# cboin1996/avddpg

Hardware: AMD Instinct MI355X
Metric: env-steps/sec + DDPG updates/sec, 4096x5-vehicle platoons (higher is better)
Workload: dtype f32-class (fp16 hi+lo operand pairs on the 16-bit matrix cores, f32 accumulate)

## Files before the change

### avddpg_amd/csrc/fsplit.hip

```cpp
#include <type_traits>

#include "fset_common.h"

namespace avd {
namespace fsplit {
using namespace fset;

struct ActorS {
    static constexpr int K = 256, KP = 256, NFT = 8, NKS = 16, LD = 264, NGT = 9, KG = 288;
    static constexpr bool critic = false;
};
struct CriticS {
    static constexpr int K = 304, KP = 320, NFT = 10, NKS = 19, LD = 312, NGT = 10, KG = 320;
    static constexpr bool critic = true;
};
constexpr int NGT_MAX = 10;

template <int I, int N, class F>
__device__ __forceinline__ void static_for(F&& f) {
    if constexpr (I < N) {
        f(std::integral_constant<int, I>{});
        static_for<I + 1, N>(f);
    }
}
// ... 17 lines not shown
    f32x2 l;
#ifdef __HIP_DEVICE_COMPILE__
    asm("v_fma_mix_f32 %0, -%1, 1.0, %2 op_sel:[0,0,0] op_sel_hi:[1,0,0]" : "=v"(l[0]) : "v"(hi), "v"(a));
    asm("v_fma_mix_f32 %0, -%1, 1.0, %2 op_sel:[1,0,0] op_sel_hi:[1,0,0]" : "=v"(l[1]) : "v"(hi), "v"(b));
#else
    l[0] = a - (float)h[0], l[1] = b - (float)h[1];
#endif
    lo = __builtin_bit_cast(unsigned, __builtin_convertvector(l, f16x2));
}
__device__ __forceinline__ void split1h(float x, f16& hi, f16& lo) {
    hi = (f16)x;
    lo = (f16)(x - (float)hi);
}
template <class V>
__device__ __forceinline__ void pin16(V& x) {
#pragma unroll
    for (int q = 0; q < 2; ++q) {
        float a = x[8 * q], b = x[8 * q + 1], c = x[8 * q + 2], d = x[8 * q + 3], e = x[8 * q + 4], f = x[8 * q + 5], g = x[8 * q + 6], h = x[8 * q + 7];
        asm volatile("" : "+v"(a), "+v"(b), "+v"(c), "+v"(d), "+v"(e), "+v"(f), "+v"(g), "+v"(h));
        x[8 * q] = a, x[8 * q + 1] = b, x[8 * q + 2] = c, x[8 * q + 3] = d, x[8 * q + 4] = e, x[8 * q + 5] = f, x[8 * q + 6] = g, x[8 * q + 7] = h;
    }
}
__device__ __forceinline__ f16x8 fragh(unsigned a, unsigned b, unsigned c, unsigned d) {
    uint4 o;
    o.x = a, o.y = b, o.z = c, o.w = d;
    return __builtin_bit_cast(f16x8, o);
}
__device__ __forceinline__ f32x16 mfmah(f16x8 a, f16x8 b, f32x16 c) {
    return __builtin_amdgcn_mfma_f32_32x32x16_f16(a, b, c, 0, 0, 0);
}
__device__ __forceinline__ f16x8 make_xh(float x0, float x1, float x2, float x3, int h) {
    f16 a0, a1, a2, a3, l0, l1, l2, l3;
    split1h(x0, a0, l0), split1h(x1, a1, l1), split1h(x2, a2, l2), split1h(x3, a3, l3);
    const f16 one = (f16)1.f, zero = (f16)0.f;
    f16x8 v;
    v[0] = a0, v[1] = a1, v[2] = a2, v[3] = a3;
    v[4] = h ? one : l0, v[5] = h ? one : l1, v[6] = h ? zero : l2, v[7] = h ? zero : l3;
    return v;
}
__device__ __forceinline__ f16x8 make_wh(float w0, float w1, float w2, float w3, float b, float sc, int h) {
    f16 a0, a1, a2, a3, l0, l1, l2, l3, bh, bl;
    split1h(sc * w0, a0, l0), split1h(sc * w1, a1, l1), split1h(sc * w2, a2, l2), split1h(sc * w3, a3, l3), split1h(sc * b, bh, bl);
    const f16 zero = (f16)0.f;
    f16x8 v;
    v[0] = h ? l0 : a0, v[1] = h ? l1 : a1, v[2] = h ? l2 : a2, v[3] = h ? l3 : a3;
    v[4] = h ? bh : a0, v[5] = h ? bl : a1, v[6] = h ? bh : a2, v[7] = h ? zero : a3;
    return v;
}
__device__ __forceinline__ f16x8 make_xg(float x0, float x1, float x2, float x3, float g, int h) {
    f16 a0, a1, a2, a3, l0, l1, l2, l3, gh, gl;
    split1h(x0, a0, l0), split1h(x1, a1, l1), split1h(x2, a2, l2), split1h(x3, a3, l3), split1h(g, gh, gl);
    const f16 zero = (f16)0.f;
    f16x8 v;
    v[0] = a0, v[1] = a1, v[2] = a2, v[3] = a3;
    v[4] = h ? gh : l0, v[5] = h ? gh : l1, v[6] = h ? gl : l2, v[7] = h ? zero : l3;
    return v;
}

template <int S>
__device__ __forceinline__ void load_x(const float* xa, long row, float (&x)[4]) {
    if (S == 4) {
        const float4 v = *(const float4*)(xa + 4 * row);
        x[0] = v.x, x[1] = v.y, x[2] = v.z, x[3] = v.w;
    } else {
#pragma unroll
        for (int k = 0; k < 4; ++k) x[k] = k < S ? xa[S * row + k] : 0.f;
    }
}

__host__ __device__ constexpr int wpos(int f) { return (f & ~12) | ((f & 4) << 1) | ((f & 8) >> 1); }

struct NetP {
    const float* th;
    long th_stride;
    const f16* Whi;
    const f16* Wlo;
    const f16* Wchi;
    const f16* Wclo;
    const f16x8* wf1h;
    const float* vec;
    const unsigned* wap;
};

struct PackArgs {
    const float* x[2];
    const float* extra[2];
    f16x8* outh[2];
    long rows;
};
__device__ __forceinline__ void front_flag(unsigned* wave_flags, bool hit) {
    const bool any = __ballot(hit) != 0;
    if ((threadIdx.x & 63) == 0) wave_flags[threadIdx.x >> 6] = any;
}
template <int S>
__device__ __forceinline__ void pack_x_role(const PackArgs& a, int which, long bx, unsigned* wave_flags) {
    const float* x = a.x[which];
    const float* extra = a.extra[which];
    const bool extra_is_action = which == 0;
    const long i = bx * 256 + threadIdx.x;
    bool nf = false;
    if (i < 2 * a.rows) {
        float v[4];
        load_x<S>(x, i >> 1, v);
        nf = not_finite(v[0]) || not_finite(v[1]) || not_finite(v[2]) || not_finite(v[3]);
        nf = nf || fmaxf(fmaxf(fabsf(v[0]), fabsf(v[1])), fmaxf(fabsf(v[2]), fabsf(v[3]))) >= F16_OVERFLOW;
        if (!(i & 1)) {
            const float e = extra[i >> 1];
            nf = nf || not_finite(e) || (extra_is_action && fabsf(e) >= F16_OVERFLOW);
        }
        a.outh[which][i] = make_xh(v[0], v[1], v[2], v[3], (int)(i & 1));
    }
    front_flag(wave_flags, nf);
}

struct PrepArgs {
    avd_mlp_layout L;
    int S;
    const float *theta, *stats, *theta_t, *stats_t;
    f16 *Whi[4], *Wlo[4];
    f16 *Wchi[4], *Wclo[4];
    f16x8* wf1h[4];
    float* vec[4];
    unsigned* wap;
    unsigned* smax;
    int* bad;
    unsigned* fflag;
    int n_fflag;
};
constexpr int SCALE_SLICES = 16;
__device__ __forceinline__ float pow2_for(float mx) {
    int e = 0;
    if (mx > 0.f && !not_finite(mx)) (void)frexpf(mx, &e);
    int k = 13 - e;
    k = k < -14 ? -14 : (k > 30 ? 30 : k);
    return ldexpf(1.f, k);
}
__device__ __forceinline__ void scale_role(const PrepArgs& a, int net, int set, int slice, int n_sets) {
    __shared__ float red[256], red2[256], c3a[H2], inva[CriticS::K];
    const int tid = threadIdx.x;
    const bool critic = net & 1, target = net >= 2;
    const avd_mlp_layout& L = a.L;
    const float* th = (target ? a.theta_t : a.theta) + (long)set * L.theta_size + (critic ? L.actor_size : 0);
    const float* st = (target ? a.stats_t : a.stats) + (long)set * L.stats_size;
    const int K = critic ? CriticS::K : ActorS::K, oW2 = critic ? L.cW2 : L.aW2;
    const int og2 = critic ? L.cg3 : L.ag2, omv2 = critic ? L.cmv3 : L.amv2, oW3 = critic ? L.cW3 : L.aW3;
    if (tid < H2) c3a[tid] = fabsf((1.0f / sqrtf(st[omv2 + tid] + BN_EPS)) * th[og2 + tid] * th[oW3 + tid]);
    for (int f = tid; f < K; f += 256) {
        int og, omv, ff = f;
        if (!critic) og = L.ag1, omv = L.amv1;
        else if (f < H1) og = L.cgs, omv = L.cmvs;
        else og = L.cga, omv = L.cmva, ff = f - H1;
        inva[f] = fabsf((1.0f / sqrtf(st[omv + ff] + BN_EPS)) * th[og + ff]);
    }
    __syncthreads();
    const int total = K * H2, per = (total + SCALE_SLICES - 1) / SCALE_SLICES, lo = slice * per, hi = min(total, lo + per);
    float m = 0.f, m2 = 0.f;
    for (int i = lo + tid; i < hi; i += 256) {
        const float w = fabsf(th[oW2 + i]);
        m = fmaxf(m, inva[i / H2] * w);
        m2 = fmaxf(m2, c3a[i % H2] * w);
    }
    red[tid] = m, red2[tid] = m2;
    __syncthreads();
    for (int o = 128; o > 0; o >>= 1) {
        if (tid < o) red[tid] = fmaxf(red[tid], red[tid + o]), red2[tid] = fmaxf(red2[tid], red2[tid + o]);
        __syncthreads();
    }
    if (tid == 0) {
        unsigned* dst = a.smax + (((long)net * n_sets + set) * SCALE_SLICES + slice) * 2;
        dst[0] = __float_as_uint(red[0]);
        dst[1] = __float_as_uint(red2[0]);
    }
}
__global__ __launch_bounds__(320) void prep_kernel(const PrepArgs a) {
    __shared__ float red[320];
    const int n = blockIdx.x, net = blockIdx.y, set = blockIdx.z, f = threadIdx.x;
    const bool critic = net & 1, target = net >= 2;
    const avd_mlp_layout& L = a.L;
    const float* th = (target ? a.theta_t : a.theta) + (long)set * L.theta_size + (critic ? L.actor_size : 0);
    const float* st = (target ? a.stats_t : a.stats) + (long)set * L.stats_size;
    const int K = critic ? CriticS::K : ActorS::K, KP = critic ? CriticS::KP : ActorS::KP;
    const int oW2 = critic ? L.cW2 : L.aW2, ob2 = critic ? L.cb2 : L.ab2, oW3 = critic ? L.cW3 : L.aW3, ob3 = critic ? L.cb3 : L.ab3;
    const int og2 = critic ? L.cg3 : L.ag2, obe2 = critic ? L.cbe3 : L.abe2, omm2 = critic ? L.cmm3 : L.amm2, omv2 = critic ? L.cmv3 : L.amv2;
    const float inv2n = (1.0f / sqrtf(st[omv2 + n] + BN_EPS)) * th[og2 + n], c3n = inv2n * th[oW3 + n];
    const unsigned* smax = a.smax + ((long)net * gridDim.z + set) * SCALE_SLICES * 2;
    unsigned mx = 0, mxc = 0;
#pragma unroll
    for (int sl = 0; sl < SCALE_SLICES; ++sl) mx = max(mx, smax[2 * sl]), mxc = max(mxc, smax[2 * sl + 1]);
    const float SW = pow2_for(__uint_as_float(mx)), SWC = pow2_for(__uint_as_float(mxc));
    if (net == 0 && set == 0)
        for (int w = n * 320 + f; w < a.n_fflag; w += H2 * 320)
            if (a.fflag[w]) atomicOr(a.bad, 1);
    float shw = 0.f;
    if (f < KP) {
        float w = 0.f, inv = 0.f;
// ... 15 lines not shown
            a.Whi[net][at] = hi, a.Wlo[net][at] = lo;
        }
        if (!target) {
            f16 hi, lo;
            const float wc = SWC * (c3n * w);
            if (fabsf(wc) >= F16_OVERFLOW) atomicOr(a.bad, 1);
            split1h(wc, hi, lo);
            const long at = ((long)set * KP + f) * H2 + n;
            a.Wchi[net][at] = hi, a.Wclo[net][at] = lo;
        }
    }
    red[f] = shw;
    __syncthreads();
    if (f < 64) red[f] += red[f + 256];
    __syncthreads();
    for (int o = 128; o > 0; o >>= 1) {
        if (f < o) red[f] += red[f + o];
        __syncthreads();
    }
    float* vec = a.vec[net] + (long)set * VEC;
    if (f == 0) {
        if (n == 0) vec[2 * H2 + 1] = SW, vec[2 * H2 + 2] = SWC;
        vec[n] = th[ob2 + n] + red[0];
        vec[H2 + n] = c3n;
        if (not_finite(vec[n]) || not_finite(c3n) || not_finite(th[ob3])) atomicOr(a.bad, 1);
    }
    if (n == 0) {
        __syncthreads();
        float v = 0.f;
        if (f < H2) {
            const float inv2 = (1.0f / sqrtf(st[omv2 + f] + BN_EPS)) * th[og2 + f];
            v = (th[obe2 + f] - st[omm2 + f] * inv2) * th[oW3 + f];
        }
        red[f] = v;
        __syncthreads();
        for (int o = 64; o > 0; o >>= 1) {
            if (f < o) red[f] += red[f + o];
            __syncthreads();
        }
        if (f == 0) vec[2 * H2] = th[ob3] + red[0];
    }
}
__device__ __forceinline__ bool prep1_role(const PrepArgs& a, int ft, int net, int set, int lane) {
    const int r = lane & 31, h = lane >> 5;
    bool hit = false;
    const bool critic = net & 1, target = net >= 2;
    const avd_mlp_layout& L = a.L;
    const float* th = (target ? a.theta_t : a.theta) + (long)set * L.theta_size + (critic ? L.actor_size : 0);
    const int K = critic ? CriticS::K : ActorS::K;
    const int f = 32 * ft + r;
    float w[4] = {0.f, 0.f, 0.f, 0.f}, b = 0.f;
    if (f == K) {
        b = 1.f;
    } else if (f < K) {
        if (critic && ft >= 8) {
            w[0] = th[L.cWa + (f - H1)], b = th[L.cba + (f - H1)];
        } else {
            const float* W = th + (critic ? L.cWs : L.aW1);
#pragma unroll
            for (int k = 0; k < 4; ++k) w[k] = k < a.S ? W[k * H1 + f] : 0.f;
            b = th[(critic ? L.cbs : L.ab1) + f];
        }
        if (not_finite(w[0]) || not_finite(w[1]) || not_finite(w[2]) || not_finite(w[3]) || not_finite(b)) hit = true;
        if (S1 * fmaxf(fmaxf(fabsf(w[0]), fabsf(w[1])), fmaxf(fmaxf(fabsf(w[2]), fabsf(w[3])), fabsf(b))) >= F16_OVERFLOW) hit = true;
    }
    a.wf1h[net][((long)set * NGT_MAX + ft) * 64 + lane] = make_wh(w[0], w[1], w[2], w[3], b, S1, h);
    if (net == 1 && ft == 0 && lane < 48) {
        const int hl = lane / 24, hh = (lane / 12) & 1, ks = (lane / 4) % 3, m = lane & 3;
        unsigned v = 0;
#pragma unroll
        for (int e = 0; e < 2; ++e) {
            const int jj = 2 * m + e, fa = 16 * ks + 8 * (jj >> 2) + 4 * hh + (jj & 3);
            f16 hi, lo;
            split1h(S1 * th[L.cWa + fa], hi, lo);
            v |= (unsigned)__builtin_bit_cast(unsigned short, hl ? lo : hi) << (16 * e);
        }
        a.wap[(long)set * 48 + lane] = v;
    }
    return hit;
}

struct FrontArgs {
    PrepArgs pa;
    PackArgs pk;
    float* grads;
    long n_grads;
    int n_sets, n_scale, n_prep1, n_zero, n_pack;
};
constexpr int ZERO_PER_BLOCK = 4096;
template <int S>
__global__ __launch_bounds__(256) void front_kernel(const FrontArgs a) {
    int b = blockIdx.x;
    if (b < a.n_scale) {
        scale_role(a.pa, b & 3, (b >> 2) % a.n_sets, (b >> 2) / a.n_sets, a.n_sets);
        return;
    }
    b -= a.n_scale;
    if (b < a.n_prep1) {
        const int q = 4 * b + (threadIdx.x >> 6);
        bool hit = false;
        if (q < NGT_MAX * 4 * a.n_sets) hit = prep1_role(a.pa, q % NGT_MAX, (q / NGT_MAX) & 3, q / (NGT_MAX * 4), threadIdx.x & 63);
        front_flag(a.pa.fflag + 4 * (long)b, hit);
        return;
    }
    b -= a.n_prep1;
    if (b < a.n_zero) {
        if (b == 0 && threadIdx.x == 0) *a.pa.bad = 0;
        const long base = (long)b * ZERO_PER_BLOCK + threadIdx.x;
#pragma unroll
        for (int k = 0; k < ZERO_PER_BLOCK / 256; ++k)
            if (base + 256 * k < a.n_grads) a.grads[base + 256 * k] = 0.f;
        return;
    }
    b -= a.n_zero;
    const int which = b >= a.n_pack;
    pack_x_role<S>(a.pk, which, b - which * a.n_pack, a.pa.fflag + 4 * ((long)a.n_prep1 + b));
}

enum HeadMode { OUT_TANH = 0, OUT_TD = 1, HEAD_BOTH = 5, OUT_TANH_SAVE = 6 };
struct HeadArgs {
    unsigned long long* stamp;
    NetP net;
    int n_agents, n_sets;
    const f16x8* xf;
    const float* act;
    const float* act2;
    const float* r;
    const float* yin;
    const float* aw;
    float* out;
    unsigned* sm;
    float* g3;
    float* dmu;
    float* part_s;
    float* part_s2;
    float* part_m;
    float* tz;
    float gamma, high, inv_n;
    int* bad;
    int abl;
};
#ifndef HEAD_FAST
#define HEAD_FAST 5
#define HEAD_SLOW 3
#endif

template <int S, class NET, int MODE, bool HP = false, class... H>
__global__ __launch_bounds__(NT) void head_kernel(const HeadArgs p, H... hp) {
    constexpr int K = NET::K, NKS = NET::NKS, NFT = NET::NFT, LD = NET::LD;
    constexpr int NTH = NT;
    constexpr bool BOTH = (MODE == HEAD_BOTH);
    static_assert(!BOTH || NET::critic, "HEAD_BOTH is a critic mode");
    __shared__ __attribute__((aligned(16))) f16 wimg[2][H2 * LD];
    __shared__ __attribute__((aligned(16))) float b2s[H2];
    __shared__ __attribute__((aligned(16))) float c3s[H2];
    __shared__ __attribute__((aligned(16))) unsigned waps[BOTH ? 48 : 4];
    const int tid = threadIdx.x, w = tid >> 6, lane = tid & 63, r = lane & 31, h = lane >> 5, q = w >> 1, rh = w & 1;
    const int set = blockIdx.x % p.n_sets, j0 = blockIdx.x / p.n_sets, J = gridDim.x / p.n_sets, P = p.n_agents / p.n_sets;
    for (int i = tid; i < 2 * H2 * (K / 8); i += NTH) {
        const int hl = i / (H2 * (K / 8)), rem = i - hl * (H2 * (K / 8)), n = rem / (K / 8), c = rem - n * (K / 8);
        const f16* src = (hl ? p.net.Wlo : p.net.Whi) + ((long)set * H2 + n) * K + 8 * c;
        *(uint4*)(&wimg[hl][n * LD + 8 * c]) = *(const uint4*)src;
    }
    const float* vec = p.net.vec + (long)set * VEC;
    const float SW = vec[2 * H2 + 1], sc = SW * S1, isc = 1.f / sc;
    if (tid < H2) b2s[tid] = vec[tid] * sc, c3s[tid] = vec[H2 + tid] * isc;
    if (BOTH && tid < 48) waps[tid] = p.net.wap[(long)set * 48 + tid];
    const float d3 = vec[2 * H2];
    const f16x8* wf1 = p.net.wf1h + (long)set * NGT_MAX * 64 + lane;
    const f32x16 zero16 = {};
#ifdef AVD_STAMP
    unsigned long long hacc[4] = {0, 0, 0, 0}, hlast = __builtin_amdgcn_s_memtime();
    const unsigned long long hstart = hlast;
#define HSTAMP(i) { const unsigned long long t_ = __builtin_amdgcn_s_memtime(); hacc[i] += t_ - hlast; hlast = t_; }
#else
#define HSTAMP(i)
#endif
    float Dacc = 0.f, Lacc = 0.f, Dacc2 = 0.f, Lacc2 = 0.f, gmax = 0.f;
    unsigned watch = 0;
    auto look = [&](float x) {
        unsigned u = __float_as_uint(x);
        asm volatile("" : "+v"(u));
        u &= 0x7fffffffu;
        watch = watch > u ? watch : u;
    };
    __syncthreads();

    const int ntile = j0 < P ? (P - j0 + J - 1) / J : 0;
    const int row = 32 * rh + r;
    f16x8 nx = {};
    float na = 0.f, nb = 0.f, ny = 0.f, nw = 1.f;
    auto fetch_in = [&](int k) {
        const int agent = (j0 + k * J) * p.n_sets + set;
        const long ri = (long)agent * TILE + row;
        nx = p.xf[2 * ri + h];
        if (NET::critic) na = p.act[ri];
        if (BOTH) nb = p.act2[ri];
        if (MODE == OUT_TD) ny = p.r[ri];
        if (BOTH) ny = p.yin[ri];
        if (BOTH && p.aw) nw = p.aw[agent];
    };
    const f16* whi0 = &wimg[0][r * LD + 8 * h];
    const f16* wlo0 = &wimg[1][r * LD + 8 * h];
    constexpr int NSEQ = BOTH ? 8 : NFT;
    HSTAMP(3);
    constexpr int FAST = HEAD_FAST, SLOW = HEAD_SLOW, PERIOD = 2 * (FAST + SLOW);
    const int qs = __builtin_amdgcn_readfirstlane(q);
    const int cnt = qs < 2 ? FAST : SLOW, start = qs < 2 ? qs * FAST : 2 * FAST + (qs - 2) * SLOW;
    int k = start, pos = 0;
    auto next_tile = [&](int kk, int pp) { return pp + 1 == cnt ? kk + PERIOD - cnt + 1 : kk + 1; };
    if (k < ntile) fetch_in(k);
    for (int ui = 0; k < ntile; ++ui, k = next_tile(k, pos), pos = pos + 1 == cnt ? 0 : pos + 1) {
        const int agent = (j0 + k * J) * p.n_sets + set;
        const long ri = (long)agent * TILE + row;
        const f16x8 xs = nx, xa = make_xh(na, 0.f, 0.f, 0.f, h), xb = BOTH ? make_xh(nb, 0.f, 0.f, 0.f, h) : xa;
        const float ty = ny, tw = nw;
        if (next_tile(k, pos) < ntile) fetch_in(next_tile(k, pos));
        f32x16 acc[4];
#pragma unroll
        for (int t = 0; t < 4; ++t)
#pragma unroll
            for (int g = 0; g < 4; ++g) {
                const float4 b = *(const float4*)(b2s + 32 * t + 8 * g + 4 * h);
                acc[t][4 * g] = b.x, acc[t][4 * g + 1] = b.y, acc[t][4 * g + 2] = b.z, acc[t][4 * g + 3] = b.w;
            }
        unsigned ph[8], pl[8];
        auto split16 = [&](const f32x16& p1) {
            if (FSPLIT_ABL(p.abl) & 4) {
#pragma unroll
                for (int m = 0; m < 8; ++m) ph[m] = __float_as_uint(p1[2 * m]), pl[m] = __float_as_uint(p1[2 * m + 1]);
                return;
            }
#pragma unroll
            for (int m = 0; m < 8; ++m) split2h(relu(p1[2 * m]), relu(p1[2 * m + 1]), ph[m], pl[m]);
        };
        auto zdot_t = [&](f32x16& a, int t) {
            float zp = 0.f;
#pragma unroll
            for (int g = 0; g < 4; ++g) {
                const float4 c = *(const float4*)(c3s + 32 * t + 8 * g + 4 * h);
                const float cc[4] = {c.x, c.y, c.z, c.w};
#pragma unroll
                for (int j = 0; j < 4; ++j) {
                    a[4 * g + j] = relu(a[4 * g + j]);
                    zp = fmaf(a[4 * g + j], cc[j], zp);
                }
            }
            return zp;
        };
        auto zdot_nd = [&](const f32x16& a, int t) {
            float zp = 0.f;
#pragma unroll
            for (int g = 0; g < 4; ++g) {
                const float4 c = *(const float4*)(c3s + 32 * t + 8 * g + 4 * h);
                const float cc[4] = {c.x, c.y, c.z, c.w};
#pragma unroll
                for (int j = 0; j < 4; ++j) zp = fmaf(relu(a[4 * g + j]), cc[j], zp);
            }
            return zp;
        };
        auto mask_t = [&](const f32x16& a) {
            unsigned b = 0;
#pragma unroll
            for (int g = 0; g < 4; ++g)
#pragma unroll
                for (int j = 0; j < 4; ++j) b |= a[4 * g + j] > 0.f ? 1u << (4 * g + (j >> 1) + 16 * (j & 1)) : 0u;
            return b;
        };
        auto mask_store = [&](const unsigned (&b)[4], unsigned* dst) {
            const auto s0 = __builtin_amdgcn_permlane32_swap(b[0], b[2], false, false);
            const auto s1 = __builtin_amdgcn_permlane32_swap(b[1], b[3], false, false);
            uint2 o;
            o.x = s0[0] | (s0[1] << 2), o.y = s1[0] | (s1[1] << 2);
            *(uint2*)(dst + 2 * h) = o;
        };
        auto out_z = [&](f32x16 (&ac)[4]) {
            float zp = 0.f;
#pragma unroll
            for (int t = 0; t < 4; ++t) zp += zdot_t(ac[t], t);
            zp += __shfl_xor(zp, 32);
            return d3 + zp;
        };
        split16(mfmah(wf1[0], xs, zero16));
        f16x8 wfn = wf1[64];
        f16x8 wg[2][2][2];
        auto read_group = [&](int g, f16x8 (&dst)[2][2]) {
            const int ks = g >> 1, th = g & 1;
#pragma unroll
            for (int tt = 0; tt < 2; ++tt) {
                dst[tt][0] = *(const f16x8*)(whi0 + 32 * (2 * th + tt) * LD + 16 * ks);
                dst[tt][1] = *(const f16x8*)(wlo0 + 32 * (2 * th + tt) * LD + 16 * ks);
            }
        };
        read_group(0, wg[0]);
        auto tile = [&](auto si_c, f32x16 (&ac)[4]) {
            constexpr int si = decltype(si_c)::value;
            constexpr int ft = si;
            f32x16 p1n = zero16;
// ... 82 lines not shown
            }
            __builtin_amdgcn_sched_barrier(0);
            f16x8 mh[3], ml[3];
#pragma unroll
            for (int tl = 0; tl < 2; ++tl) {
                const f32x16 pa = mfmah(wf1[64 * (8 + tl)], xa, zero16), pm = mfmah(wf1[64 * (8 + tl)], xb, zero16);
                unsigned dh[8], dl[8], mk[8];
#pragma unroll
                for (int m = 0; m < 4 * (2 - tl); ++m) {
                    split2h(relu(pm[2 * m]) - relu(pa[2 * m]), relu(pm[2 * m + 1]) - relu(pa[2 * m + 1]), dh[m], dl[m]);
                    mk[m] = (pm[2 * m] > 0.f ? 0xffffu : 0u) | (pm[2 * m + 1] > 0.f ? 0xffff0000u : 0u);
                }
#pragma unroll
                for (int ss = 0; ss < 2 - tl; ++ss) {
                    const int kk = 2 * tl + ss;
                    fh[kk] = fragh(dh[4 * ss], dh[4 * ss + 1], dh[4 * ss + 2], dh[4 * ss + 3]);
                    fl[kk] = fragh(dl[4 * ss], dl[4 * ss + 1], dl[4 * ss + 2], dl[4 * ss + 3]);
                    const uint4 ch = *(const uint4*)(waps + (0 * 2 + h) * 12 + 4 * kk), cl = *(const uint4*)(waps + (1 * 2 + h) * 12 + 4 * kk);
                    mh[kk] = fragh(ch.x & mk[4 * ss], ch.y & mk[4 * ss + 1], ch.z & mk[4 * ss + 2], ch.w & mk[4 * ss + 3]);
                    ml[kk] = fragh(cl.x & mk[4 * ss], cl.y & mk[4 * ss + 1], cl.z & mk[4 * ss + 2], cl.w & mk[4 * ss + 3]);
                }
            }
            act_sweep(acc);
            look(acc[0][0]);
            float zq = 0.f;
            unsigned pos[2] = {0u, 0u};
#pragma unroll
            for (int t = 0; t < 4; ++t) {
                zq += zdot_nd(acc[t], t);
#pragma unroll
                for (int i = 0; i < 16; ++i) pos[t >> 1] |= acc[t][i] > 0.f ? 1u << (16 * (t & 1) + i) : 0u;
            }
            zq += __shfl_xor(zq, 32);
            asm volatile("" : "+v"(pos[0]), "+v"(pos[1]));
#pragma unroll
            for (int kk = 0; kk < 3; ++kk) fh[kk] = mh[kk], fl[kk] = ml[kk];
#pragma unroll
            for (int t = 0; t < 4; ++t) acc[t] = zero16;
            act_sweep(acc);
            float sum = 0.f;
#pragma unroll
            for (int t = 0; t < 4; ++t)
#pragma unroll
                for (int g = 0; g < 4; ++g) {
                    const float4 c = *(const float4*)(c3s + 32 * t + 8 * g + 4 * h);
                    const float cc[4] = {c.x, c.y, c.z, c.w};
#pragma unroll
                    for (int j = 0; j < 4; ++j) sum += (pos[t >> 1] >> (16 * (t & 1) + 4 * g + j) & 1u) ? cc[j] * acc[t][4 * g + j] : 0.f;
                }
            sum += __shfl_xor(sum, 32);
            const float g3b = -p.inv_n * tw;
            if (h == 0) p.dmu[ri] = g3b * sum, Dacc2 += g3b, Lacc2 += d3 + zq;
            continue;
        }
        look(acc[0][0]);
        const float z = out_z(acc);
        if (MODE == OUT_TANH) {
            const float o = tanhf(z) * p.high;
            if (h == 0) p.out[ri] = o;
        } else if (MODE == OUT_TANH_SAVE) {
            const float t = tanhf(z);
            if (h == 0) p.out[ri] = t * p.high, p.tz[ri] = t;
            unsigned mb[4];
#pragma unroll
            for (int tt = 0; tt < 4; ++tt) mb[tt] = mask_t(acc[tt]);
            mask_store(mb, p.sm + ri * 4);
        } else {
            if constexpr (HP) {
                if (h == 0) p.out[ri] = ty + hp_of(set, hp...).gamma * z;
            } else {
                if (h == 0) p.out[ri] = ty + p.gamma * z;
            }
        }
        HSTAMP(2);
#ifdef AVD_STAMP
        if (blockIdx.x == 16 && lane == 0 && p.stamp && (w == 0 || w == 4) && ui < 28)
            p.stamp[64 + (w >> 2) * 28 + ui] = hlast - hstart;
#endif
    }
#ifdef AVD_STAMP
    if (blockIdx.x == 16 && lane == 0 && p.stamp)
        for (int i = 0; i < 4; ++i) p.stamp[w * 8 + i] = hacc[i];
#endif
    if (watch >= 0x7f800000u) atomicOr(p.bad, 1);
    if (BOTH) {
#pragma unroll
        for (int o = 1; o < 32; o <<= 1) {
            Dacc += __shfl_xor(Dacc, o), Lacc += __shfl_xor(Lacc, o);
            Dacc2 += __shfl_xor(Dacc2, o), Lacc2 += __shfl_xor(Lacc2, o);
        }
#pragma unroll
        for (int o = 1; o < 64; o <<= 1) gmax = fmaxf(gmax, __shfl_xor(gmax, o));
        if (lane == 0) {
            const long slot = (long)blockIdx.x * 8 + w;
            p.part_m[slot] = gmax;
            p.part_s[slot * 2] = Dacc, p.part_s[slot * 2 + 1] = Lacc;
            p.part_s2[slot * 2] = Dacc2, p.part_s2[slot * 2 + 1] = Lacc2;
        }
    }
}

struct SeedArgs {
    int n_agents, n_sets;
    const float *dmu, *tz;
    float high;
    float *g3, *part_m, *part_s;
};
__global__ __launch_bounds__(NT) void actor_seed_kernel(const SeedArgs p) {
    const int tid = threadIdx.x, w = tid >> 6, lane = tid & 63;
    const int set = blockIdx.x % p.n_sets, j0 = blockIdx.x / p.n_sets, J = gridDim.x / p.n_sets, P = p.n_agents / p.n_sets;
    float gmax = 0.f, D = 0.f;
    for (int pi = j0 + w * J; pi < P; pi += 8 * J) {
        const long ri = (long)(pi * p.n_sets + set) * TILE + lane;
        const float t = p.tz[ri], g = p.dmu[ri] * p.high * (1.f - t * t);
        p.g3[ri] = g;
        gmax = fmaxf(gmax, fabsf(g));
        D += g;
    }
#pragma unroll
    for (int o = 1; o < 64; o <<= 1) gmax = fmaxf(gmax, __shfl_xor(gmax, o)), D += __shfl_xor(D, o);
    if (lane == 0) {
        p.part_m[(long)blockIdx.x * 8 + w] = gmax;
        p.part_s[((long)blockIdx.x * 8 + w) * 2] = D, p.part_s[((long)blockIdx.x * 8 + w) * 2 + 1] = 0.f;
    }
}

__device__ __forceinline__ float set_gscale(const float* part_m, int set, int n_sets, int J, float* red) {
    const int tid = threadIdx.x;
    float m = 0.f;
    for (int i = tid; i < J * 8; i += NT) m = fmaxf(m, part_m[((long)(i >> 3) * n_sets + set) * 8 + (i & 7)]);
#pragma unroll
    for (int o = 1; o < 64; o <<= 1) m = fmaxf(m, __shfl_xor(m, o));
    if ((tid & 63) == 0) red[tid >> 6] = m;
    __syncthreads();
    m = fmaxf(fmaxf(fmaxf(red[0], red[1]), fmaxf(red[2], red[3])), fmaxf(fmaxf(red[4], red[5]), fmaxf(red[6], red[7])));
    int e = 0;
    if (m > 0.f && !not_finite(m)) (void)frexpf(m, &e);
    const int k = e > 100 ? -100 : (e < -100 ? 100 : -e);
    return __uint_as_float(__builtin_amdgcn_readfirstlane(__float_as_uint(ldexpf(1.f, k))));
}

__device__ __forceinline__ unsigned mask_pair(unsigned d, int j, unsigned mj) { return __umul24(d & (0x10001u << j), mj); }
__device__ __forceinline__ void mask_chunk16(unsigned w, int c, unsigned m, uint4& lo, uint4& hi) {
    const unsigned d = w >> (8 * (c & 1));
    lo.x = mask_pair(d, 0, m), lo.y = mask_pair(d, 1, m >> 1), lo.z = mask_pair(d, 2, m >> 2), lo.w = mask_pair(d, 3, m >> 3);
    hi.x = mask_pair(d, 4, m >> 4), hi.y = mask_pair(d, 5, m >> 5), hi.z = mask_pair(d, 6, m >> 6), hi.w = mask_pair(d, 7, m >> 7);
}
__device__ __forceinline__ unsigned mask_one(float g3, bool signed_) { return signed_ && g3 < 0.f ? 0xbc00u : 0x3c00u; }

struct DwArgs {
    NetP net;
    int n_agents, n_sets;
    const float* x;
    const float* act;
    const float* g3;
    const float* part_m;
    const unsigned* sm;
    float* partG;
    int abl;
    unsigned long long* stamp;
};
template <int S, class NET>
__global__ __launch_bounds__(NT) void dw_kernel(const DwArgs p) {
    constexpr int KG = NET::KG, LDZ = 160;
    constexpr int XC = NET::critic ? 2 : 1;
    __shared__ __attribute__((aligned(16))) f16 smimg[2][TILE * LDZ];
    __shared__ __attribute__((aligned(16))) f16x8 fq[2][TILE * 2];
// ... 434 lines not shown
    const float gv = gsc * VSH, vs = gsc * swc * VSH;
    const float* th = p.net.th + (long)set * p.net.th_stride;
    const float wa = f < HA ? th[p.L_cWa + f] : 0.f, ba = f < HA ? th[p.L_cba + f] : 0.f;
    float Sa = 0.f, Sb = 0.f;
    const int ntile = j0 < P ? (P - j0 + J - 1) / J : 0;
    uint4 mA = {}, mB = {};
    float gA = 0.f, aA = 0.f, gB = 0.f, aB = 0.f;
#define DXA_FETCH(k_, m_, g_, a_)                                                                                   \
    {                                                                                                               \
        const long r0_ = (long)((j0 + (k_) * J) * p.n_sets + set) * TILE + 32 * rh;                                 \
        m_ = *(const uint4*)(p.sm + (r0_ + r) * 4);                                                                 \
        g_ = p.g3[r0_ + r], a_ = p.act[r0_ + r];                                                                    \
    }
#define DXA_PUT(buf_, g_, a_)                                                                                       \
    {                                                                                                               \
        if (h == 0) ga[w][buf_][0][r] = fabsf(g_) * gv, ga[w][buf_][1][r] = a_;                                     \
        __builtin_amdgcn_fence(__ATOMIC_RELEASE, "wavefront");                                                      \
        __builtin_amdgcn_wave_barrier();                                                                            \
    }
    auto unit = [&](int buf, const uint4 mw, float g) {
        f32x16 dc = zero16;
        const unsigned m = mask_one(g, true);
        const unsigned mwt[4] = {mw.x >> (4 * h), mw.y >> (4 * h), mw.z >> (4 * h), mw.w >> (4 * h)};
#pragma unroll
        for (int s = 0; s < 8; ++s) {
            const unsigned d = mwt[s >> 1] >> (8 * (s & 1));
            const f16x8 af = fragh(mask_pair(d, 0, m), mask_pair(d, 1, m >> 1), mask_pair(d, 2, m >> 2), mask_pair(d, 3, m >> 3));
            dc = mfmah(af, wch[s], dc), dc = mfmah(af, wcl[s], dc);
        }
        float sa = 0.f, sb = 0.f;
#pragma unroll
        for (int q = 0; q < 4; ++q) {
            const float4 gq = *(const float4*)(&ga[w][buf][0][8 * q + 4 * h]), aq = *(const float4*)(&ga[w][buf][1][8 * q + 4 * h]);
            const float gg[4] = {gq.x, gq.y, gq.z, gq.w}, av[4] = {aq.x, aq.y, aq.z, aq.w};
#pragma unroll
            for (int j = 0; j < 4; ++j) {
                const float m = fmaf(av[j], wa, ba) > 0.f ? dc[4 * q + j] * gg[j] : 0.f;
                sa = fmaf(m, av[j], sa);
                sb += m;
            }
        }
        Sa += sa, Sb += sb;
        __builtin_amdgcn_fence(__ATOMIC_ACQ_REL, "wavefront");
        __builtin_amdgcn_wave_barrier();
    };
    if (par < ntile) DXA_FETCH(par, mA, gA, aA);
    if (par + 2 < ntile) DXA_FETCH(par + 2, mB, gB, aB);
    for (int k = par; k < ntile; k += 4) {
        DXA_PUT(0, gA, aA);
        {
            const uint4 mc = mA;
            const float gc = gA;
            if (k + 4 < ntile) DXA_FETCH(k + 4, mA, gA, aA);
            unit(0, mc, gc);
        }
        if (k + 2 < ntile) {
            DXA_PUT(1, gB, aB);
            const uint4 mc = mB;
            const float gc = gB;
            if (k + 6 < ntile) DXA_FETCH(k + 6, mB, gB, aB);
            unit(1, mc, gc);
        }
    }
#undef DXA_FETCH
#undef DXA_PUT
    comb[w][lane][0] = Sa, comb[w][lane][1] = Sb;
    __syncthreads();
    if (rh == 0 && par == 0 && h == 0) {
        const int ws[4] = {w, w + 1, w + 4, w + 5};
        float t[2] = {0.f, 0.f};
#pragma unroll
        for (int i = 0; i < 4; ++i)
#pragma unroll
            for (int c = 0; c < 2; ++c) t[c] += comb[ws[i]][r][c] + comb[ws[i]][32 + r][c];
        const float ivs = 1.f / vs;
        float* pv = p.partV + ((long)blockIdx.x * KP + 32 * ft + r) * 16;
#pragma unroll
        for (int c = 0; c < 9; ++c) pv[c] = c == 0 ? t[0] * ivs : (c == 8 ? t[1] * ivs : 0.f);
    }
}

struct Plan {
    int grid, J;
    size_t Whi[4], Wlo[4], Wchi[2], Wclo[2], wf1h[4], vec[4], wap, a2, y, mu, dmu, g3, sm, sma, tz, t1p, s2raw, xfs, xfs2, partHs[3], partM[2],
        partV[2], partG[2], bad, smax, fflag, total;
    int n_prep1, n_pack, n_fflag;
};
static Plan make_plan(int n_agents, int n_sets) {
    Plan pl;
    const int P = n_agents / n_sets;
    int J = cu_count() / n_sets;
    if (const char* e = AVD_DIAG_ENV("FSPLIT_J")) J = atoi(e);
    if (J < 1) J = 1;
    if (J > P) J = P;
    pl.J = J, pl.grid = J * n_sets;
    size_t o = 0;
    auto take = [&](size_t bytes) {
        const size_t at = o;
        o += (bytes + 255) / 256 * 256;
        return at;
    };
    for (int i = 0; i < 4; ++i) {
        const int K = (i & 1) ? CriticS::K : ActorS::K, KP = (i & 1) ? CriticS::KP : ActorS::KP;
        pl.Whi[i] = take(sizeof(f16) * (size_t)n_sets * H2 * K), pl.Wlo[i] = take(sizeof(f16) * (size_t)n_sets * H2 * K);
        pl.vec[i] = take(sizeof(float) * (size_t)n_sets * VEC);
        pl.wf1h[i] = take(16 * (size_t)n_sets * NGT_MAX * 64);
        if (i < 2) pl.Wchi[i] = take(sizeof(f16) * (size_t)n_sets * KP * H2), pl.Wclo[i] = take(sizeof(f16) * (size_t)n_sets * KP * H2);
    }
    pl.wap = take(4 * (size_t)n_sets * 48);
    const size_t rows = (size_t)n_agents * TILE;
    pl.a2 = take(4 * rows), pl.y = take(4 * rows), pl.mu = take(4 * rows), pl.dmu = take(4 * rows), pl.g3 = take(4 * rows);
    pl.sm = take(16 * rows);
    pl.sma = take(16 * rows);
    pl.tz = take(4 * rows);
    pl.t1p = take(2 * 4 * (size_t)n_sets * CriticS::K * H2), pl.s2raw = take(2 * 4 * (size_t)n_sets * H2);
    pl.xfs = take(32 * rows), pl.xfs2 = take(32 * rows);
    for (int i = 0; i < 2; ++i) {
        const int KP = i ? CriticS::KP : ActorS::KP, KG = i ? CriticS::KG : ActorS::KG;
        pl.partM[i] = take(4 * (size_t)pl.grid * 8);
        pl.partV[i] = take(4 * (size_t)pl.grid * KP * 16);
        pl.partG[i] = take(4 * (size_t)pl.grid * KG * H2);
    }
    for (int i = 0; i < 3; ++i) pl.partHs[i] = take(4 * (size_t)pl.grid * 8 * 2);
    pl.n_prep1 = (NGT_MAX * 4 * n_sets + 3) / 4, pl.n_pack = (int)((2 * rows + 255) / 256);
    pl.n_fflag = 4 * (pl.n_prep1 + 2 * pl.n_pack);
    pl.bad = take(sizeof(int));
    pl.smax = take(sizeof(unsigned) * 4 * (size_t)n_sets * SCALE_SLICES * 2);
    pl.fflag = take(sizeof(unsigned) * (size_t)pl.n_fflag);
    pl.total = o;
    return pl;
}
static int check_shape(const avd_mlp_layout* L, int n_agents, int n_sets, const char* who) {
    AVD_REQUIRE(L, "%s: null layout", who);
    if (L->H1 != H1 || L->H2 != H2 || L->Ha != HA || L->A != 1 || (L->S != 3 && L->S != 4) || L->B != TILE) {
        set_error("%s: serves the reference widths only (layer1 256, layer2 128, action layer 48, A = 1, S in {3, 4}, B = 64); "
                  "got H1=%d H2=%d Ha=%d A=%d S=%d B=%d (avd_learn_shared_bf16 takes other widths)",
                  who, L->H1, L->H2, L->Ha, L->A, L->S, L->B);
        return AVD_E_UNSUPPORTED;
    }
    AVD_REQUIRE(n_sets > 0 && n_sets <= 64 && n_agents > 0 && n_agents % n_sets == 0, "%s: n_agents=%d n_sets=%d", who, n_agents,
                n_sets);
    return AVD_OK;
}

enum Phase { PH_CRITIC = 1, PH_ACTOR = 2, PH_BOTH = 3 };
template <int S, class... H>
static int run(int phases, const avd_mlp_layout& L, int n_agents, int n_sets, const float* theta, const float* stats, const float* theta_t,
               const float* stats_t, const float* s, const float* a, const float* r, const float* s2, const float* aw, float gamma,
               float high, float* grads, float* losses, unsigned char* ws, const Plan& pl, hipStream_t st, H... hp) {
    PrepArgs pa;
    pa.L = L, pa.S = S, pa.theta = theta, pa.stats = stats, pa.theta_t = theta_t, pa.stats_t = stats_t;
    pa.wap = (unsigned*)(ws + pl.wap), pa.bad = (int*)(ws + pl.bad), pa.smax = (unsigned*)(ws + pl.smax);
    pa.fflag = (unsigned*)(ws + pl.fflag), pa.n_fflag = pl.n_fflag;
    NetP net[4];
    for (int i = 0; i < 4; ++i) {
        const bool critic = i & 1, target = i >= 2;
        pa.Whi[i] = (f16*)(ws + pl.Whi[i]), pa.Wlo[i] = (f16*)(ws + pl.Wlo[i]), pa.vec[i] = (float*)(ws + pl.vec[i]);
        pa.wf1h[i] = (f16x8*)(ws + pl.wf1h[i]);
        pa.Wchi[i] = i < 2 ? (f16*)(ws + pl.Wchi[i]) : nullptr, pa.Wclo[i] = i < 2 ? (f16*)(ws + pl.Wclo[i]) : nullptr;
        NetP& n = net[i];
        n.th = (target ? theta_t : theta) + (critic ? L.actor_size : 0), n.th_stride = L.theta_size;
        n.Whi = pa.Whi[i], n.Wlo = pa.Wlo[i], n.Wchi = pa.Wchi[i], n.Wclo = pa.Wclo[i], n.wf1h = pa.wf1h[i], n.vec = pa.vec[i];
        n.wap = pa.wap;
    }
    const int P = n_agents / n_sets;
    const float inv_n = 1.0f / ((float)P * TILE);
    const long nrows = (long)n_agents * TILE;
    f16x8 *xfs = (f16x8*)(ws + pl.xfs), *xfs2 = (f16x8*)(ws + pl.xfs2);
    int* bad = (int*)(ws + pl.bad);
    float *a2 = (float*)(ws + pl.a2), *y = (float*)(ws + pl.y), *mu = (float*)(ws + pl.mu), *dmu = (float*)(ws + pl.dmu);
    float* g3 = (float*)(ws + pl.g3);
    unsigned *sm = (unsigned*)(ws + pl.sm), *sma = (unsigned*)(ws + pl.sma);
    auto F = [&](size_t off) { return (float*)(ws + off); };
    const dim3 grid(pl.grid), block(NT);
    HeadArgs h;
    h.n_agents = n_agents, h.n_sets = n_sets, h.gamma = gamma, h.high = high, h.inv_n = inv_n, h.aw = aw, h.sm = sm, h.g3 = g3, h.dmu = dmu;
    h.act2 = nullptr, h.part_s2 = nullptr, h.stamp = nullptr, h.bad = bad, h.part_m = nullptr, h.tz = F(pl.tz), h.abl = 0;
    if (const char* e = AVD_DIAG_ENV("FSPLIT_ABL")) h.abl = atoi(e);
    auto head = [&](auto kern, int ni, const f16x8* x, const float* act, const float* rr, const float* yin, float* out, float* part_s,
                    auto... extra) {
        h.net = net[ni], h.xf = x, h.act = act, h.r = rr, h.yin = yin, h.out = out, h.part_s = part_s;
        hipLaunchKernelGGL(kern, grid, block, 0, st, h, extra...);
    };
    DwArgs dw;
    dw.n_agents = n_agents, dw.n_sets = n_sets, dw.sm = sm, dw.g3 = g3, dw.x = s, dw.stamp = nullptr, dw.abl = 0;
    if (const char* e = AVD_DIAG_ENV("FSPLIT_ABL")) dw.abl = atoi(e);
#ifdef AVD_STAMP
    static unsigned long long* d_stamp = nullptr;
    if (!d_stamp) (void)hipMalloc(&d_stamp, 128 * 8);
    dw.stamp = d_stamp;
#endif
    DxArgs dx;
    dx.n_agents = n_agents, dx.n_sets = n_sets, dx.sm = sm, dx.g3 = g3, dx.xfh = xfs, dx.stamp = nullptr, dx.L_cWa = dx.L_cba = 0;
    dx.abl = dw.abl;
#ifdef AVD_STAMP
    dx.stamp = d_stamp;
#endif
    FinArgs fa;
    fa.L = L, fa.n_sets = n_sets, fa.J = pl.J, fa.S = S, fa.nrh = 1, fa.theta = theta, fa.stats = stats, fa.grads = grads, fa.losses = losses;
    fa.inv_n = inv_n, fa.partLa = F(pl.partHs[2]), fa.bad = bad;
    for (int i = 0; i < 2; ++i)
        fa.partH[i] = nullptr, fa.partHs[i] = F(pl.partHs[i]), fa.partU[i] = nullptr, fa.partV[i] = F(pl.partV[i]),
        fa.partG[i] = F(pl.partG[i]), fa.c3[i] = F(pl.vec[i]);
    fa.t1_from_g[0] = fa.t1_from_g[1] = 1, fa.t1p = F(pl.t1p), fa.s2raw = F(pl.s2raw);
    if (phases & PH_CRITIC) {
        FrontArgs fr;
        fr.pa = pa, fr.grads = grads, fr.n_grads = (long)n_sets * L.theta_size, fr.n_sets = n_sets;
        fr.pk.x[0] = s, fr.pk.extra[0] = a, fr.pk.outh[0] = xfs, fr.pk.x[1] = s2, fr.pk.extra[1] = r, fr.pk.outh[1] = xfs2, fr.pk.rows = nrows;
        fr.n_scale = 4 * n_sets * SCALE_SLICES, fr.n_prep1 = pl.n_prep1, fr.n_pack = pl.n_pack;
        fr.n_zero = (int)((fr.n_grads + ZERO_PER_BLOCK - 1) / ZERO_PER_BLOCK);
        hipLaunchKernelGGL(front_kernel<S>, dim3((unsigned)(fr.n_scale + fr.n_prep1 + fr.n_zero + 2 * fr.n_pack)), dim3(256), 0, st, fr);
        hipLaunchKernelGGL(prep_kernel, dim3(H2, 4, n_sets), dim3(320), 0, st, pa);
        head(head_kernel<S, ActorS, OUT_TANH>, 2, xfs2, nullptr, nullptr, nullptr, a2, nullptr);
        if constexpr (sizeof...(H) > 0)
            head(head_kernel<S, CriticS, OUT_TD, true, H...>, 3, xfs2, a2, r, nullptr, y, nullptr, hp...);
        else
            head(head_kernel<S, CriticS, OUT_TD>, 3, xfs2, a2, r, nullptr, y, nullptr);
        h.sm = sma;
        head(head_kernel<S, ActorS, OUT_TANH_SAVE>, 0, xfs, nullptr, nullptr, nullptr, mu, nullptr);
        h.sm = sm;
        h.act2 = mu, h.part_s2 = F(pl.partHs[2]), h.part_m = F(pl.partM[1]);
        head(head_kernel<S, CriticS, HEAD_BOTH>, 1, xfs, a, nullptr, y, nullptr, F(pl.partHs[1]));
        dw.net = net[1], dw.act = a, dw.partG = F(pl.partG[1]), dw.part_m = F(pl.partM[1]);
        hipLaunchKernelGGL((dw_kernel<S, CriticS>), grid, block, 0, st, dw);
        dx.net = net[1], dx.partV = F(pl.partV[1]), dx.act = a, dx.part_m = F(pl.partM[1]);
        hipLaunchKernelGGL((dx_kernel<S, CriticS>), grid, block, 0, st, dx);
        dx.L_cWa = L.cWa, dx.L_cba = L.cba;
        hipLaunchKernelGGL((dxa_kernel<S>), grid, block, 0, st, dx);
        if (phases == PH_CRITIC) launch_finalize(fa, st, 1, 1);
    }
    if (phases & PH_ACTOR) {
        SeedArgs sd;
        sd.n_agents = n_agents, sd.n_sets = n_sets, sd.dmu = dmu, sd.tz = F(pl.tz), sd.high = high, sd.g3 = g3, sd.part_m = F(pl.partM[0]),
        sd.part_s = F(pl.partHs[0]);
        hipLaunchKernelGGL(actor_seed_kernel, grid, block, 0, st, sd);
        dw.sm = sma, dx.sm = sma;
        dw.net = net[0], dw.act = nullptr, dw.partG = F(pl.partG[0]), dw.part_m = F(pl.partM[0]);
        hipLaunchKernelGGL((dw_kernel<S, ActorS>), grid, block, 0, st, dw);
        dx.net = net[0], dx.partV = F(pl.partV[0]), dx.act = nullptr, dx.part_m = F(pl.partM[0]), dx.L_cWa = dx.L_cba = 0;
        hipLaunchKernelGGL((dx_kernel<S, ActorS>), grid, block, 0, st, dx);
        if (phases == PH_ACTOR) launch_finalize(fa, st, 0, 1);
        else launch_finalize(fa, st, 0, 2);
    }
    return check_launch("avd_learn_set_split");
}

}
}

using namespace avd;

namespace avd { namespace fsplit {
constexpr long MFMA_PER_TILE = 2 * (200 + 238 + 200 + 314)
                               + 8 * (2 + 32 + 1 + 2 * 2 * 2)
                               + 8 * (2 + 32 + 1 + 2 * 1 * 2)
                               + 2 * 8 * (32 + 2 + 8)
                               + 4 * 16;
static_assert(MFMA_PER_TILE == 3296, "update DESIGN.md 3.4 and the count above together");
}}
extern "C" int avd_learn_set_split_mfma_count(const avd_mlp_layout* lay, int n_agents, int n_sets, unsigned long long* mfma_32x32x16) {
    int rc = fsplit::check_shape(lay, n_agents, n_sets, "avd_learn_set_split_mfma_count");
    if (rc) return rc;
    AVD_REQUIRE(mfma_32x32x16, "avd_learn_set_split_mfma_count: null pointer");
    *mfma_32x32x16 = (unsigned long long)fsplit::MFMA_PER_TILE * (unsigned long long)n_agents;
    return AVD_OK;
}

extern "C" int avd_learn_set_split_workspace(const avd_mlp_layout* lay, int n_agents, int n_sets, size_t* bytes) {
    int rc = fsplit::check_shape(lay, n_agents, n_sets, "avd_learn_set_split_workspace");
    if (rc) return rc;
    AVD_REQUIRE(bytes, "avd_learn_set_split_workspace: null pointer");
    *bytes = fsplit::make_plan(n_agents, n_sets).total;
    return AVD_OK;
}

template <class... H>
static int split_entry(int phases, const char* who, const avd_mlp_layout* lay, int n_agents, int n_sets, const float* theta, const float* stats,
                       const float* theta_t, const float* stats_t, const float* s, const float* a, const float* r, const float* s2,
                       const float* agent_weight, float gamma, float high, float* grads, float* losses, void* workspace,
                       size_t workspace_bytes, void* stream, H... hp) {
    int rc = fsplit::check_shape(lay, n_agents, n_sets, who);
    if (rc) return rc;
    const bool cr = phases & fsplit::PH_CRITIC;
    AVD_REQUIRE(theta && stats && s && grads && workspace && (!cr || (theta_t && stats_t && a && r && s2)), "%s: null pointer", who);
    const fsplit::Plan pl = fsplit::make_plan(n_agents, n_sets);
    AVD_REQUIRE(workspace_bytes >= pl.total, "%s: workspace %zu B < %zu B", who, workspace_bytes, pl.total);
    if (lay->S == 4)
        return fsplit::run<4>(phases, *lay, n_agents, n_sets, theta, stats, theta_t, stats_t, s, a, r, s2, agent_weight, gamma, high, grads,
                              losses, (unsigned char*)workspace, pl, (hipStream_t)stream, hp...);
    return fsplit::run<3>(phases, *lay, n_agents, n_sets, theta, stats, theta_t, stats_t, s, a, r, s2, agent_weight, gamma, high, grads, losses,
                          (unsigned char*)workspace, pl, (hipStream_t)stream, hp...);
}

extern "C" int avd_learn_set_split_f16x3(const avd_mlp_layout* lay, int n_agents, int n_sets, const float* theta, const float* stats,
                                          const float* theta_t, const float* stats_t, const float* s, const float* a, const float* r,
                                          const float* s2, const float* agent_weight, float gamma, float high, float* grads,
                                          float* losses, void* workspace, size_t workspace_bytes, void* stream) {
    return split_entry(fsplit::PH_BOTH, "avd_learn_set_split_f16x3", lay, n_agents, n_sets, theta, stats, theta_t, stats_t, s, a, r, s2,
                       agent_weight, gamma, high, grads, losses, workspace, workspace_bytes, stream);
}

extern "C" int avd_learn_set_split_hp_f16x3(const avd_mlp_layout* lay, int n_agents, int n_sets, const float* theta, const float* stats,
                                            const float* theta_t, const float* stats_t, const float* s, const float* a, const float* r,
// ... 30 lines not shown
```

Measured before the change: 2.123 million.

## Fuse state f16 packing into head kernels; scan only actions and rewards in front

Drops the front-kernel pass that packed s and s2 into f16 hi/lo buffers, along with the xfs2 workspace. The target head kernels now read raw f32 states and split them in registers. The actor-save head also writes the packed xfs that the later critic and backward kernels still use. The front kernel only scans actions and rewards for overflow and non-finite values, with vectorized loads. State range checks move into the actor heads, which avoids a full write and reread of the packed state buffers. The cost is redundant conversion work in the heads and a later point at which bad inputs are detected.

```diff
diff --git a/avddpg_amd/csrc/fsplit.hip b/avddpg_amd/csrc/fsplit.hip
--- a/avddpg_amd/csrc/fsplit.hip
+++ b/avddpg_amd/csrc/fsplit.hip
@@ -123,35 +123,38 @@
     const unsigned* wap;
 };
 
-struct PackArgs {
-    const float* x[2];
-    const float* extra[2];
-    f16x8* outh[2];
+struct ScanArgs {
+    const float *a, *r;
     long rows;
 };
 __device__ __forceinline__ void front_flag(unsigned* wave_flags, bool hit) {
     const bool any = __ballot(hit) != 0;
     if ((threadIdx.x & 63) == 0) wave_flags[threadIdx.x >> 6] = any;
 }
-template <int S>
-__device__ __forceinline__ void pack_x_role(const PackArgs& a, int which, long bx, unsigned* wave_flags) {
-    const float* x = a.x[which];
-    const float* extra = a.extra[which];
-    const bool extra_is_action = which == 0;
-    const long i = bx * 256 + threadIdx.x;
-    bool nf = false;
-    if (i < 2 * a.rows) {
-        float v[4];
-        load_x<S>(x, i >> 1, v);
-        nf = not_finite(v[0]) || not_finite(v[1]) || not_finite(v[2]) || not_finite(v[3]);
-        nf = nf || fmaxf(fmaxf(fabsf(v[0]), fabsf(v[1])), fmaxf(fabsf(v[2]), fabsf(v[3]))) >= F16_OVERFLOW;
-        if (!(i & 1)) {
-            const float e = extra[i >> 1];
-            nf = nf || not_finite(e) || (extra_is_action && fabsf(e) >= F16_OVERFLOW);
-        }
-        a.outh[which][i] = make_xh(v[0], v[1], v[2], v[3], (int)(i & 1));
-    }
-    front_flag(wave_flags, nf);
+constexpr unsigned F16_OVERFLOW_BITS = 0x477ff000u;
+constexpr unsigned INF_BITS = 0x7f800000u;
+__device__ __forceinline__ unsigned abs_bits(float x) {
+    unsigned u = __float_as_uint(x);
+    asm("" : "+v"(u));
+    return u & 0x7fffffffu;
+}
+constexpr int SCAN_PER_BLOCK = 1024;
+__device__ __forceinline__ void scan_role(const ScanArgs& p, long bx, unsigned* wave_flags) {
+    const long i = bx * SCAN_PER_BLOCK + 4 * threadIdx.x;
+    unsigned ma = 0, mr = 0;
+    if (i < p.rows) {
+        float va[4], vr[4];
+        if ((((unsigned long long)p.a | (unsigned long long)p.r) & 15) == 0) {
+            const float4 qa = *(const float4*)(p.a + i), qr = *(const float4*)(p.r + i);
+            va[0] = qa.x, va[1] = qa.y, va[2] = qa.z, va[3] = qa.w, vr[0] = qr.x, vr[1] = qr.y, vr[2] = qr.z, vr[3] = qr.w;
+        } else {
+#pragma unroll
+            for (int k = 0; k < 4; ++k) va[k] = p.a[i + k], vr[k] = p.r[i + k];
+        }
+#pragma unroll
+        for (int k = 0; k < 4; ++k) ma = max(ma, abs_bits(va[k])), mr = max(mr, abs_bits(vr[k]));
+    }
+    front_flag(wave_flags, ma >= F16_OVERFLOW_BITS || mr >= INF_BITS);
 }
 
 struct PrepArgs {
@@ -333,13 +336,12 @@
 
 struct FrontArgs {
     PrepArgs pa;
-    PackArgs pk;
+    ScanArgs sc;
     float* grads;
     long n_grads;
-    int n_sets, n_scale, n_prep1, n_zero, n_pack;
+    int n_sets, n_scale, n_prep1, n_zero, n_scan;
 };
 constexpr int ZERO_PER_BLOCK = 4096;
-template <int S>
 __global__ __launch_bounds__(256) void front_kernel(const FrontArgs a) {
     int b = blockIdx.x;
     if (b < a.n_scale) {
@@ -364,8 +366,7 @@
         return;
     }
     b -= a.n_zero;
-    const int which = b >= a.n_pack;
-    pack_x_role<S>(a.pk, which, b - which * a.n_pack, a.pa.fflag + 4 * ((long)a.n_prep1 + b));
+    scan_role(a.sc, b, a.pa.fflag + 4 * ((long)a.n_prep1 + b));
 }
 
 enum HeadMode { OUT_TANH = 0, OUT_TD = 1, HEAD_BOTH = 5, OUT_TANH_SAVE = 6 };
@@ -373,7 +374,10 @@
     unsigned long long* stamp;
     NetP net;
     int n_agents, n_sets;
-    const f16x8* xf;
+    union {
+        const f16x8* xf;
+        const float* xraw;
+    };
     const float* act;
     const float* act2;
     const float* r;
@@ -382,7 +386,10 @@
     float* out;
     unsigned* sm;
     float* g3;
-    float* dmu;
+    union {
+        float* dmu;
+        f16x8* xfo;
+    };
     float* part_s;
     float* part_s2;
     float* part_m;
@@ -401,6 +408,7 @@
     constexpr int K = NET::K, NKS = NET::NKS, NFT = NET::NFT, LD = NET::LD;
     constexpr int NTH = NT;
     constexpr bool BOTH = (MODE == HEAD_BOTH);
+    constexpr bool RAW = !BOTH, WATCH_X = (MODE == OUT_TANH || MODE == OUT_TANH_SAVE);
     static_assert(!BOTH || NET::critic, "HEAD_BOTH is a critic mode");
     __shared__ __attribute__((aligned(16))) f16 wimg[2][H2 * LD];
     __shared__ __attribute__((aligned(16))) float b2s[H2];
@@ -428,7 +436,7 @@
 #define HSTAMP(i)
 #endif
     float Dacc = 0.f, Lacc = 0.f, Dacc2 = 0.f, Lacc2 = 0.f, gmax = 0.f;
-    unsigned watch = 0;
+    unsigned watch = 0, watchx = 0;
     auto look = [&](float x) {
         unsigned u = __float_as_uint(x);
         asm volatile("" : "+v"(u));
@@ -440,11 +448,13 @@
     const int ntile = j0 < P ? (P - j0 + J - 1) / J : 0;
     const int row = 32 * rh + r;
     f16x8 nx = {};
+    float nxr[4] = {0.f, 0.f, 0.f, 0.f};
     float na = 0.f, nb = 0.f, ny = 0.f, nw = 1.f;
     auto fetch_in = [&](int k) {
         const int agent = (j0 + k * J) * p.n_sets + set;
         const long ri = (long)agent * TILE + row;
-        nx = p.xf[2 * ri + h];
+        if constexpr (RAW) load_x<S>(p.xraw, ri, nxr);
+        else nx = p.xf[2 * ri + h];
         if (NET::critic) na = p.act[ri];
         if (BOTH) nb = p.act2[ri];
         if (MODE == OUT_TD) ny = p.r[ri];
@@ -464,7 +474,13 @@
     for (int ui = 0; k < ntile; ++ui, k = next_tile(k, pos), pos = pos + 1 == cnt ? 0 : pos + 1) {
         const int agent = (j0 + k * J) * p.n_sets + set;
         const long ri = (long)agent * TILE + row;
-        const f16x8 xs = nx, xa = make_xh(na, 0.f, 0.f, 0.f, h), xb = BOTH ? make_xh(nb, 0.f, 0.f, 0.f, h) : xa;
+        f16x8 xs = nx;
+        if constexpr (RAW) {
+            xs = make_xh(nxr[0], nxr[1], nxr[2], nxr[3], h);
+            if constexpr (WATCH_X) watchx = max(max(watchx, abs_bits(nxr[0])), max(max(abs_bits(nxr[1]), abs_bits(nxr[2])), abs_bits(nxr[3])));
+            if constexpr (MODE == OUT_TANH_SAVE) p.xfo[2 * ri + h] = xs;
+        }
+        const f16x8 xa = make_xh(na, 0.f, 0.f, 0.f, h), xb = BOTH ? make_xh(nb, 0.f, 0.f, 0.f, h) : xa;
         const float ty = ny, tw = nw;
         if (next_tile(k, pos) < ntile) fetch_in(next_tile(k, pos));
         f32x16 acc[4];
@@ -713,7 +729,9 @@
     if (blockIdx.x == 16 && lane == 0 && p.stamp)
         for (int i = 0; i < 4; ++i) p.stamp[w * 8 + i] = hacc[i];
 #endif
-    if (watch >= 0x7f800000u) atomicOr(p.bad, 1);
+    bool hit = watch >= 0x7f800000u;
+    if constexpr (WATCH_X) hit = hit || watchx >= F16_OVERFLOW_BITS;
+    if (hit) atomicOr(p.bad, 1);
     if (BOTH) {
 #pragma unroll
         for (int o = 1; o < 32; o <<= 1) {
@@ -1314,9 +1332,9 @@
 
 struct Plan {
     int grid, J;
-    size_t Whi[4], Wlo[4], Wchi[2], Wclo[2], wf1h[4], vec[4], wap, a2, y, mu, dmu, g3, sm, sma, tz, t1p, s2raw, xfs, xfs2, partHs[3], partM[2],
+    size_t Whi[4], Wlo[4], Wchi[2], Wclo[2], wf1h[4], vec[4], wap, a2, y, mu, dmu, g3, sm, sma, tz, t1p, s2raw, xfs, partHs[3], partM[2],
         partV[2], partG[2], bad, smax, fflag, total;
-    int n_prep1, n_pack, n_fflag;
+    int n_prep1, n_scan, n_fflag;
 };
 static Plan make_plan(int n_agents, int n_sets) {
     Plan pl;
@@ -1346,7 +1364,7 @@
     pl.sma = take(16 * rows);
     pl.tz = take(4 * rows);
     pl.t1p = take(2 * 4 * (size_t)n_sets * CriticS::K * H2), pl.s2raw = take(2 * 4 * (size_t)n_sets * H2);
-    pl.xfs = take(32 * rows), pl.xfs2 = take(32 * rows);
+    pl.xfs = take(32 * rows);
     for (int i = 0; i < 2; ++i) {
         const int KP = i ? CriticS::KP : ActorS::KP, KG = i ? CriticS::KG : ActorS::KG;
         pl.partM[i] = take(4 * (size_t)pl.grid * 8);
@@ -1354,8 +1372,8 @@
         pl.partG[i] = take(4 * (size_t)pl.grid * KG * H2);
     }
     for (int i = 0; i < 3; ++i) pl.partHs[i] = take(4 * (size_t)pl.grid * 8 * 2);
-    pl.n_prep1 = (NGT_MAX * 4 * n_sets + 3) / 4, pl.n_pack = (int)((2 * rows + 255) / 256);
-    pl.n_fflag = 4 * (pl.n_prep1 + 2 * pl.n_pack);
+    pl.n_prep1 = (NGT_MAX * 4 * n_sets + 3) / 4, pl.n_scan = (int)((rows + SCAN_PER_BLOCK - 1) / SCAN_PER_BLOCK);
+    pl.n_fflag = 4 * (pl.n_prep1 + pl.n_scan);
     pl.bad = take(sizeof(int));
     pl.smax = take(sizeof(unsigned) * 4 * (size_t)n_sets * SCALE_SLICES * 2);
     pl.fflag = take(sizeof(unsigned) * (size_t)pl.n_fflag);
@@ -1398,7 +1416,7 @@
     const int P = n_agents / n_sets;
     const float inv_n = 1.0f / ((float)P * TILE);
     const long nrows = (long)n_agents * TILE;
-    f16x8 *xfs = (f16x8*)(ws + pl.xfs), *xfs2 = (f16x8*)(ws + pl.xfs2);
+    f16x8* xfs = (f16x8*)(ws + pl.xfs);
     int* bad = (int*)(ws + pl.bad);
     float *a2 = (float*)(ws + pl.a2), *y = (float*)(ws + pl.y), *mu = (float*)(ws + pl.mu), *dmu = (float*)(ws + pl.dmu);
     float* g3 = (float*)(ws + pl.g3);
@@ -1409,9 +1427,9 @@
     h.n_agents = n_agents, h.n_sets = n_sets, h.gamma = gamma, h.high = high, h.inv_n = inv_n, h.aw = aw, h.sm = sm, h.g3 = g3, h.dmu = dmu;
     h.act2 = nullptr, h.part_s2 = nullptr, h.stamp = nullptr, h.bad = bad, h.part_m = nullptr, h.tz = F(pl.tz), h.abl = 0;
     if (const char* e = AVD_DIAG_ENV("FSPLIT_ABL")) h.abl = atoi(e);
-    auto head = [&](auto kern, int ni, const f16x8* x, const float* act, const float* rr, const float* yin, float* out, float* part_s,
+    auto head = [&](auto kern, int ni, const void* x, const float* act, const float* rr, const float* yin, float* out, float* part_s,
                     auto... extra) {
-        h.net = net[ni], h.xf = x, h.act = act, h.r = rr, h.yin = yin, h.out = out, h.part_s = part_s;
+        h.net = net[ni], h.xf = (const f16x8*)x, h.act = act, h.r = rr, h.yin = yin, h.out = out, h.part_s = part_s;
         hipLaunchKernelGGL(kern, grid, block, 0, st, h, extra...);
     };
     DwArgs dw;
@@ -1438,19 +1456,19 @@
     if (phases & PH_CRITIC) {
         FrontArgs fr;
         fr.pa = pa, fr.grads = grads, fr.n_grads = (long)n_sets * L.theta_size, fr.n_sets = n_sets;
-        fr.pk.x[0] = s, fr.pk.extra[0] = a, fr.pk.outh[0] = xfs, fr.pk.x[1] = s2, fr.pk.extra[1] = r, fr.pk.outh[1] = xfs2, fr.pk.rows = nrows;
-        fr.n_scale = 4 * n_sets * SCALE_SLICES, fr.n_prep1 = pl.n_prep1, fr.n_pack = pl.n_pack;
+        fr.sc.a = a, fr.sc.r = r, fr.sc.rows = nrows;
+        fr.n_scale = 4 * n_sets * SCALE_SLICES, fr.n_prep1 = pl.n_prep1, fr.n_scan = pl.n_scan;
         fr.n_zero = (int)((fr.n_grads + ZERO_PER_BLOCK - 1) / ZERO_PER_BLOCK);
-        hipLaunchKernelGGL(front_kernel<S>, dim3((unsigned)(fr.n_scale + fr.n_prep1 + fr.n_zero + 2 * fr.n_pack)), dim3(256), 0, st, fr);
+        hipLaunchKernelGGL(front_kernel, dim3((unsigned)(fr.n_scale + fr.n_prep1 + fr.n_zero + fr.n_scan)), dim3(256), 0, st, fr);
         hipLaunchKernelGGL(prep_kernel, dim3(H2, 4, n_sets), dim3(320), 0, st, pa);
-        head(head_kernel<S, ActorS, OUT_TANH>, 2, xfs2, nullptr, nullptr, nullptr, a2, nullptr);
+        head(head_kernel<S, ActorS, OUT_TANH>, 2, s2, nullptr, nullptr, nullptr, a2, nullptr);
         if constexpr (sizeof...(H) > 0)
-            head(head_kernel<S, CriticS, OUT_TD, true, H...>, 3, xfs2, a2, r, nullptr, y, nullptr, hp...);
+            head(head_kernel<S, CriticS, OUT_TD, true, H...>, 3, s2, a2, r, nullptr, y, nullptr, hp...);
         else
-            head(head_kernel<S, CriticS, OUT_TD>, 3, xfs2, a2, r, nullptr, y, nullptr);
-        h.sm = sma;
-        head(head_kernel<S, ActorS, OUT_TANH_SAVE>, 0, xfs, nullptr, nullptr, nullptr, mu, nullptr);
-        h.sm = sm;
+            head(head_kernel<S, CriticS, OUT_TD>, 3, s2, a2, r, nullptr, y, nullptr);
+        h.sm = sma, h.xfo = xfs;
+        head(head_kernel<S, ActorS, OUT_TANH_SAVE>, 0, s, nullptr, nullptr, nullptr, mu, nullptr);
+        h.sm = sm, h.dmu = dmu;
         h.act2 = mu, h.part_s2 = F(pl.partHs[2]), h.part_m = F(pl.partM[1]);
         head(head_kernel<S, CriticS, HEAD_BOTH>, 1, xfs, a, nullptr, y, nullptr, F(pl.partHs[1]));
         dw.net = net[1], dw.act = a, dw.partG = F(pl.partG[1]), dw.part_m = F(pl.partM[1]);
```

New measurement: 2.142 million, median of 6. No clear change (+0.9%).
